# seanrjohnson/protein_gibbs_sampler

Measured on AMD Instinct MI355X. Metric: sampled positions/sec (whole node), ESM-1b L=256 B=256 Gibbs, higher is better.
Workload: dtype bf16; 1 GPU; ESM_sampler ESM-1b (33 layers, d=1280) Gibbs: 256 chains in total, 256 per GPU x L=256 (T=258), P=25 positions per chain per iteration, mask=True top_k=0 temperature=1.0 burnin=inf; bf16 MFMA operands, fp32 accumulate + fp32 residual stream; synthetic weights N(0,0.025), embeddings N(0,0.3), LayerNorm jitter 0.1 (logit std ~10); global_batch=256, seq_len=256, parallelism=chains sharded 1-way (contiguous blocks), 1 RCCL all-gather at the end, n_layers=33

## Files before the change

protein_gibbs_sampler_amd/csrc/attention.hip:

```cpp
#include <stdlib.h>

#include "attn_frag.h"

PG_OPS_BEGIN


#ifdef PG_ATT_PROF
__device__ unsigned long long* pg_att_prof;
#define PG_T(slot, i)                                                                                              \
  do {                                                                                                             \
    if ((slot) < 8 && (threadIdx.x & 63) == 0)                                                                     \
      pg_att_prof[(((size_t)blockIdx.x * 4 + (threadIdx.x >> 6)) * 8 + (slot)) * 8 + (i)] = __builtin_readcyclecounter(); \
  } while (0)
#else
#define PG_T(slot, i)
#endif

constexpr int attention_occupancy(int maxkb, int hd) { return hd == 64 ? (maxkb <= 18 ? 2 : 1) : 2; }
constexpr int attention_resident32(int kb) { return kb <= 20 ? 4 : (kb <= 26 ? 3 : 2); }
template <int MAXKB, bool PADMASK, bool BIASKV = false, bool SPLIT = false, int HD = 64>
__global__ __launch_bounds__(256, attention_occupancy(MAXKB, HD)) void attention_kernel(const bf16_t* __restrict__ qkv, bf16_t* __restrict__ ctx, int T,
                                                       int H, int ld_qkv_, int ld_ctx_, int k_off, int v_off,
                                                       SeqLayout sl, const int32_t* __restrict__ key_tok, int pad_idx,
                                                       const bf16_t* __restrict__ bias_kv, int split_from = 0, int split = 1) {
  constexpr int ROW = HD * 2, NKK = HD / 32, NDB = HD / 16;
  __shared__ __attribute__((aligned(16))) char smem[2 * MAXKB * 16 * ROW + (PADMASK ? MAXKB * 16 : 0)];
  char* Ks = smem;
  char* Vs = smem + MAXKB * 16 * ROW;
  char* padf = smem + 2 * MAXKB * 16 * ROW;

  const int tid = threadIdx.x, lane = tid & 63, wave = tid >> 6;
  PG_T(7, 0);
  int pair = blockIdx.x, qb_first = wave, qb_step = 4;
  if (SPLIT && (int)blockIdx.x >= split_from) {
    const int u = blockIdx.x - split_from;
    pair = split_from + u / split;
    qb_first = u % split + split * wave;
    qb_step = 4 * split;
  }
  const int seq = pair / H, h = pair % H;
  const size_t row0 = (size_t)(seq / sl.inner_count) * sl.outer_rows + (size_t)(seq % sl.inner_count) * sl.inner_rows;
  const size_t ld_qkv = (size_t)ld_qkv_ * sl.row_step, ld_ctx = (size_t)ld_ctx_ * sl.row_step;
  const bf16_t* base = qkv + row0 * ld_qkv_ + h * HD;
  const int Tk = T + (BIASKV ? 1 : 0);
  constexpr int nkc = MAXKB / 2;

  stage_kv<MAXKB * 16, 256, BIASKV, HD>(Ks, Vs, tid, base, ld_qkv, k_off, v_off, 0, T, bias_kv + h * HD, bias_kv + (H + h) * HD);
  if (PADMASK) {
    for (int key = tid; key < MAXKB * 16; key += 256)
      padf[key] = (key < T && key_tok[row0 + (size_t)key * sl.row_step] == pad_idx) ? 1 : 0;
  }
  PG_T(7, 1);
  __syncthreads();
  PG_T(7, 2);

  const int fr = lane & 15, fq = lane >> 4;
  const int nqb = (T + 15) >> 4;
  bf16x8 qf[NKK], qn[NKK];
  auto load_q = [&](int qb, bf16x8 (&dst)[NKK]) {
    int qrow = qb * 16 + fr;
    if (qrow >= T) qrow = T - 1;
#pragma unroll
    for (int kk = 0; kk < NKK; ++kk) dst[kk] = *(const bf16x8*)(base + (size_t)qrow * ld_qkv + kk * 32 + fq * 8);
  };
  if (qb_first < nqb) load_q(qb_first, qf);
  for (int qb = qb_first; qb < nqb; qb += qb_step) {
    if (qb + qb_step < nqb) load_q(qb + qb_step, qn);
    PG_T(qb >> 2, 0);

    f32x4 st[MAXKB];
    {
      constexpr int CH = (MAXKB % 6 == 0) ? 6 : (MAXKB % 4 == 0 ? 4 : 2);
      bf16x8 kbuf[2][CH][NKK];
      auto load_chunk = [&](int ch, bf16x8 (&dst)[CH][NKK]) {
#pragma unroll
        for (int u = 0; u < CH; ++u) {
#if defined(PG_ATT_PROF) && PG_ATT_ABL == 1
          const int krow = (ch * CH + (u > 0 ? 0 : u)) * 16 + fr;
          if (u > 0) { for (int kk = 0; kk < NKK; ++kk) dst[u][kk] = dst[0][kk]; continue; }
#else
          const int krow = (ch * CH + u) * 16 + fr;
#endif
#pragma unroll
          for (int kk = 0; kk < NKK; ++kk) dst[u][kk] = k_frag<HD>(Ks, krow, kk, fq);
        }
      };
// ... 42 lines not shown
#pragma unroll
        for (int db = 0; db < NDB; ++db) {
#if defined(PG_ATT_PROF) && PG_ATT_ABL == 2
          if (db > 0) { dst[db] = dst[0]; continue; }
#endif
#pragma unroll
          for (int hh = 0; hh < 2; ++hh) dst[db].h[hh] = vt_half<HD>(Vs, (2 * c + hh) * 16, db, fr, fq);
        }
      };
      load_v(0, vbuf[0]);
      if (nkc > 1) load_v(1, vbuf[1]);
#pragma unroll
      for (int c = 0; c < nkc; ++c) {
        if (c + 2 < nkc) load_v(c + 2, vbuf[(c + 2) % 3]);
        const bf16x8 pf = p_frag(st[2 * c], st[2 * c + 1]);
        __builtin_amdgcn_sched_barrier(0);
#pragma unroll
        for (int db = 0; db < NDB; ++db) o[db] = mfma_op16(vbuf[c % 3][db].v, pf, o[db]);
        __builtin_amdgcn_sched_barrier(0);
      }
    }
    PG_T(qb >> 2, 3);
    const int q = qb * 16 + fr;
    if (q < T) store_ctx(o, inv, ctx + row0 * ld_ctx_ + (size_t)q * ld_ctx + h * HD + fq * 4);
    qf[0] = qn[0];
    if constexpr (NKK == 2) qf[1] = qn[1];
    PG_T(qb >> 2, 4);
  }
  PG_T(7, 3);
}

template <int MAXKB, int OCC, bool PADMASK, bool BIASKV, int HD = 64>
__global__ __launch_bounds__(256, OCC) void attention_long_kernel(const bf16_t* __restrict__ qkv, bf16_t* __restrict__ ctx, int T,
                                                               int H, int ld_qkv_, int ld_ctx_, int k_off, int v_off,
                                                               SeqLayout sl, int n_qchunk, const int32_t* __restrict__ key_tok_,
                                                               int pad_idx, const bf16_t* __restrict__ bias_kv_) {
  const int32_t* __restrict__ key_tok = PADMASK ? key_tok_ : nullptr;
  const bf16_t* __restrict__ bias_kv = BIASKV ? bias_kv_ : nullptr;
  constexpr int tpad = MAXKB * 16, nkc = MAXKB / 2;
  constexpr int ROW = HD * 2, NKK = HD / 32, NDB = HD / 16;
  __shared__ __attribute__((aligned(16))) char smem[2 * tpad * ROW + (PADMASK ? tpad : 0)];
  char* Ks = smem;
  char* Vs = smem + tpad * ROW;
  char* padf = smem + 2 * tpad * ROW;
  const int tid = threadIdx.x, lane = tid & 63, wave = tid >> 6;
  const int qc = blockIdx.x % n_qchunk, sh = blockIdx.x / n_qchunk;
  const int seq = sh / H, h = sh % H;
// ... 111 lines not shown
  dim3 grid((unsigned)(n_seq * H)), block(256);
  static const int fine_ladder = env_int("PGIBBS_ATTN_LADDER", 1);
  const int kb = attention_rung(T + (bias_kv ? 1 : 0), fine_ladder && !bias_kv);
  static const int split_on = env_int("PGIBBS_ATTN_SPLIT", 1);
  int split_from = 0, split = 1;
  if (split_on && !key_tok && !bias_kv && sl.row_step == 1 && T >= 64 && kb) {
    const long pairs = n_seq * H, slots = (long)device_cu_count() * (head_dim == 64 ? (kb <= 20 ? 2 : 1) : attention_resident32(kb));
    const long rem = pairs % slots;
    const int nqb = (T + 15) / 16;
    int sp = rem ? (int)(slots / rem) : 1;
    if (sp > 4) sp = 4;
    if (sp > nqb / 4) sp = nqb / 4;
    if (sp >= 2) {
      split = sp;
      split_from = (int)(pairs - rem);
      grid = dim3((unsigned)(split_from + rem * sp));
    }
  }
  switch (kb) {
#define PG_RUNG(KB)                                                                                                          \
  case KB:                                                                                                                   \
    if (head_dim == 64)                                                                                                      \
      launch_rung<KB, 64>(key_tok, bias_kv, split > 1, grid, s, qkv, ctx, T, H, ld_qkv, ld_ctx, k_off, v_off, sl, key_tok,   \
                          pad_idx, bias_kv, split_from, split);                                                              \
    else                                                                                                                     \
      launch_rung<KB, 32>(key_tok, false, split > 1, grid, s, qkv, ctx, T, H, ld_qkv, ld_ctx, k_off, v_off, sl, key_tok,     \
                          pad_idx, bias_kv, split_from, split);                                                              \
    break;
    PG_RUNG(2) PG_RUNG(4) PG_RUNG(6) PG_RUNG(8) PG_RUNG(10) PG_RUNG(12) PG_RUNG(14) PG_RUNG(16) PG_RUNG(18) PG_RUNG(20)
    PG_RUNG(22) PG_RUNG(24) PG_RUNG(26) PG_RUNG(28) PG_RUNG(30) PG_RUNG(32) PG_RUNG(34) PG_RUNG(36)
#undef PG_RUNG
    default: {
      const int n_qchunk = (T + 63) / 64;
      if (n_seq * H * n_qchunk > 0x7fffffff) return fail(1, "attention: too many sequences");
      const dim3 g((unsigned)(n_seq * H * n_qchunk));
#define PG_ATT_LONG(P, B) hipLaunchKernelGGL((attention_long_kernel<18, 2, P, B>), g, block, 0, s, qkv, ctx, T, H, ld_qkv, ld_ctx, k_off, v_off, sl, n_qchunk, key_tok, pad_idx, bias_kv)
#define PG_ATT_LONG32(P) hipLaunchKernelGGL((attention_long_kernel<18, 2, P, false, 32>), g, block, 0, s, qkv, ctx, T, H, ld_qkv, ld_ctx, k_off, v_off, sl, n_qchunk, key_tok, pad_idx, bias_kv)
      if (head_dim == 32) {
        if (key_tok) PG_ATT_LONG32(true);
        else PG_ATT_LONG32(false);
      } else if (key_tok && bias_kv) PG_ATT_LONG(true, true);
      else if (key_tok) PG_ATT_LONG(true, false);
      else if (bias_kv) PG_ATT_LONG(false, true);
      else PG_ATT_LONG(false, false);
#undef PG_ATT_LONG32
#undef PG_ATT_LONG
    }
  }
  PG_HIP(hipGetLastError());
  return 0;
}

PG_OPS_END
```

protein_gibbs_sampler_amd/csrc/engine.h:

```cpp
#pragma once
#include <map>
#include <string>
#include <vector>

#include "kernels.h"

namespace pg {

#define OPS(fn, ...) (precision == PG_PREC_F16 ? opf16::fn(__VA_ARGS__) : opbf16::fn(__VA_ARGS__))

struct DevBuf {
  void* p = nullptr;
  size_t bytes = 0;
  int ensure(size_t need, hipStream_t s);
  void release();
  template <typename T> T* as() const { return (T*)p; }
};

struct Prof {
  struct Rec { int cls; hipEvent_t a, b; std::string kernels; };
  bool on = false;
  std::vector<Rec> recs;
  std::vector<hipEvent_t> pool;
  size_t used = 0;
// ... 24 lines not shown
struct MsaLayer {
  LnW ln_row, ln_col;
  DenseW row_qkv, row_out, col_qkv, col_out;
  FfnW ffn;
  DenseW col_qkv_hm;
};

struct Engine {
  pg_model_config cfg;
  int device = 0;
  int precision = 0;
  hipStream_t own_stream = nullptr, stream = nullptr;
  std::vector<void*> owned;

  float *embed = nullptr, *pos = nullptr, *msa_pos = nullptr, *embed_out = nullptr;
  float embed_scale() const { return cfg.arch == PG_ARCH_ESM1 ? sqrtf((float)cfg.d_model) : 1.0f; }
  LnW ln_before, ln_after, head_ln;
  DenseW head_dense;
  float* head_bias = nullptr;
  std::vector<EsmLayer> esm_layers;
  std::vector<MsaLayer> msa_layers;

  DevBuf x, h, qkv, ctx, ffn, sel_h, sel_g, logits, d_tokens, d_idx, d_samp_tok, d_samp_logits, d_rowmap, scratch;
  DevBuf x_sel, ctx_sel, h_sel, ffn_sel;
  int resid_gemm_ln(const bf16_t* a, const DenseW& W, float* x, int M_rows, int64_t M_real, int lda, const LnW& ln, bf16_t* h,
                    float* ws = nullptr, size_t ws_bytes = 0, int prof_class = PC_GEMM, int colmajor_R = 0, int colmajor_C = 0);
  DevBuf tmp_idx, tmp_out;
  DevBuf splitk;
  bool esm_pad_in_batch = false;
  float* splitk_ws(int rows, int n, int K, int64_t batch_rows);
  int64_t job_items = 0;
  int64_t order_items = 0;
  int64_t job_batch(int64_t B) const { return order_items > 0 ? order_items : (job_items > B ? job_items : B); }
  int64_t batch_rows_for(int64_t B, int64_t rows_per_item) const { return job_batch(B) * rows_per_item; }
  int64_t batch_rows = 0;
  int sel_gemm_rows(int64_t n_sel, int64_t Np) const;
  DevBuf d_iter;
  PgChainLayerW* chain_layers = nullptr;
  DevBuf chain_sync, chain_part;
  unsigned* chain_err = nullptr;
  int chain_check();
  bool chain_disabled = false, chain_retry = false;
  struct ChainCall {
    int32_t* d_tok; int B, T; const int32_t* d_idx; int n_iters, P; pg_sample_params sp; float* lg; int32_t* st; size_t snap_off;
  };
  std::vector<ChainCall> chain_log;
  bool chain_replay_ok = false;
// ... 10 lines not shown
  int64_t stat_graph_captures = 0, stat_graph_replays = 0;
  DevBuf ffn_f32, scores;
  bool strict() const { return precision == PG_PREC_FP32; }
  bool esm1() const { return cfg.arch == PG_ARCH_ESM1; }
  bool esm2() const { return cfg.arch == PG_ARCH_ESM2; }
  bool esm_family() const { return cfg.arch == PG_ARCH_ESM1B || cfg.arch == PG_ARCH_ESM1 || cfg.arch == PG_ARCH_ESM2; }
  int head_dim = 64;
  float* rope_tab = nullptr;
  int rope_rows = 0;
  int rope(void* qkv_rows, int64_t M, int T);
  int dense3(const bf16_t* x3, const DenseW& W, float* out, int Mp, bool accumulate);
  int dense3_gelu(const bf16_t* x3, const DenseW& W, int Mp, const DenseW* next = nullptr);
  bool dense3_wants_dup(const DenseW& W, int Mp, bool gelu = false) const;
  Prof prof;

  ~Engine();
  int init(const pg_model_config* c, const pg_tensor* tensors, int n_tensors, int device_ordinal, int precision);

  int size_activations(int64_t Mp);
  int ffn_block(const DenseW& out, const FfnW& F, const LnW* next_ln, int Mi, int64_t M);
  int ffn_strict(const FfnW& F, int Mi, int64_t M);
  bool prune_last(int64_t n_draws, int64_t token_rows) const;
  int pruned_tail(const DenseW& out, const FfnW& F, const int32_t* sel_idx, const int32_t* sel_row_map, int P, int width, int64_t n_sel,
                  const int32_t* d_iter, int Ni, bool ln_in_gemm);
  int esm_trunk(const int32_t* d_tok, int B, int T, const int32_t* sel_idx, int P, int64_t n_sel, const int32_t* d_iter);
  int head(const int32_t* d_idx, const int32_t* d_row_map, int P, int width, int64_t n_sel, float* d_logits,
           const float* x_src = nullptr);
  int trunk(const int32_t* d_tok, int B, int R, int C, const int32_t* sel_idx = nullptr, const int32_t* sel_row_map = nullptr, int P = 0,
            int64_t n_sel = 0, const int32_t* d_iter = nullptr);
  int masked_logits(int32_t* d_tok, int B, int R, int C, const int32_t* idx, const int32_t* mask_map, const int32_t* sel_map,
                    int64_t n_rows, int P, bool mask, int mask_idx, float* lg, const int32_t* dit = nullptr);
  int esm_gibbs_device(int32_t* d_tok, int B, int T, const int32_t* d_idx, int n_iters, int P, const pg_sample_params* sp,
                       float* d_samp_logits, int32_t* d_samp_tok);
  int msa_trunk(const int32_t* d_tok, int B, int R, int C, const int32_t* sel_idx, const int32_t* sel_row_map, int P, int64_t n_sel);
  int msa_gibbs_device(int32_t* d_tok, int B, int R, int C, const int32_t* d_idx, int n_iters, int P,
                       const pg_sample_params* sp, float* d_samp_logits, int32_t* d_samp_tok);
  int msa_single_device(int32_t* d_tok, int B, int R, int C, int mask_row, int target_row, const int32_t* d_step_idx,
                        const int32_t* step_sample_flag_host, int n_steps, int P_max, const pg_sample_params* sp,
                        float* d_samp_logits, int32_t* d_samp_tok);

  template <typename F> int timed(int cls, F&& f);
};

std::vector<float> rope_table(int rows, int hd = 64);

struct TensorMap {
  std::map<std::string, const pg_tensor*> m;
// ... 9 lines not shown
```

protein_gibbs_sampler_amd/csrc/engine.hip:

```cpp
#include "engine.h"

#include <math.h>
#include <stdlib.h>
#include <string.h>

#include "gemm_epilogue.h"

namespace pg {

static thread_local std::string g_last_error;
void set_error(const std::string& msg) { g_last_error = msg; }
int fail(int code, const std::string& msg) {
  g_last_error = msg;
  return code;
}
const char* last_error_cstr() { return g_last_error.c_str(); }

static thread_local std::string g_noted;
void note_kernel(const char* label, long tiles, int splits) {
  if (g_noted.size() > 512) return;
  if (!g_noted.empty()) g_noted += " + ";
  g_noted += label;
  if (tiles >= 0) g_noted += " " + std::to_string(tiles) + "t";
  if (splits > 1) g_noted += " x" + std::to_string(splits) + "k";
// ... 50 lines not shown
  int rc = f();
  PG_HIP(hipEventRecord(b, stream));
  prof.recs.push_back({cls, a, b, noted_kernels()});
  return rc;
}

const float* TensorMap::get(const std::string& name, int64_t numel, std::string& err) const {
  auto it = m.find(name);
  if (it == m.end()) {
    err = "missing tensor '" + name + "'";
    return nullptr;
  }
  if (it->second->numel != numel) {
    err = "tensor '" + name + "' has " + std::to_string(it->second->numel) + " elements, expected " + std::to_string(numel);
    return nullptr;
  }
  return it->second->data;
}

Engine::~Engine() {
  if (device >= 0) (void)hipSetDevice(device);
  for (void* p : owned) (void)hipFree(p);
  DevBuf* bufs[] = {&x, &h, &qkv, &ctx, &ffn, &sel_h, &sel_g, &logits, &d_tokens, &d_idx, &d_samp_tok, &d_samp_logits,
                    &d_rowmap, &scratch, &d_iter, &tmp_idx, &tmp_out, &x_sel, &ctx_sel, &h_sel, &ffn_sel, &ffn_f32, &scores, &splitk,
                    &chain_sync, &chain_part, &chain_snap};
  for (DevBuf* b : bufs) b->release();
  if (chain_err) (void)hipHostFree(chain_err);
  if (range_err) (void)hipHostFree(range_err);
  prof.destroy();
  if (graph_exec) (void)hipGraphExecDestroy(graph_exec);
  if (own_stream) (void)hipStreamDestroy(own_stream);
}

namespace {
struct Uploader {
  Engine* e;
  const TensorMap* tm;
  const int precision;
  std::string err;

  float* f32(const std::string& name, int64_t numel) {
    const float* src = tm->get(name, numel, err);
    if (!src) return nullptr;
    void* d = nullptr;
    if (hipMalloc(&d, (size_t)numel * 4) != hipSuccess) { err = "hipMalloc failed for " + name; return nullptr; }
    e->owned.push_back(d);
    if (hipMemcpy(d, src, (size_t)numel * 4, hipMemcpyHostToDevice) != hipSuccess) { err = "H2D failed for " + name; return nullptr; }
// ... 319 lines not shown
  int rc;
  if ((rc = timed(PC_LN, [&] { return OPS(launch_layernorm_bf16, stream, X, F.ln.g, F.ln.b, H3, M, cfg.d_model, cfg.layer_norm_eps, true, 0, 0, dense3_wants_dup(F.fc1, Mi, true)); }))) return rc;
  if ((rc = dense3_gelu(H3, F.fc1, Mi, &F.fc2))) return rc;
  return dense3(ffn.as<bf16_t>(), F.fc2, X, Mi, true);
}

int Engine::ffn_block(const DenseW& out, const FfnW& F, const LnW* next_ln, int Mi, int64_t M) {
  const int d = cfg.d_model, f = cfg.d_ffn;
  float* X = x.as<float>();
  bf16_t* Hh = h.as<bf16_t>();
  bf16_t* FFN = ffn.as<bf16_t>();
  int rc;
  if ((rc = resid_gemm_ln(ctx.as<bf16_t>(), out, X, Mi, M, d, F.ln, Hh, nullptr, 0, PC_GEMM_OUT))) return rc;
  if ((rc = timed(PC_GEMM_FC1, [&] { return OPS(launch_gemm_bf16, stream, Hh, F.fc1.w, F.fc1.b, FFN, Mi, f, d, d, d, f, EPI_BF16_GELU, nullptr, 0, (int)M); }))) return rc;
  if (next_ln) return resid_gemm_ln(FFN, F.fc2, X, Mi, M, f, *next_ln, Hh, splitk_ws(Mi, d, f, batch_rows), splitk.bytes, PC_GEMM_FC2);
  return timed(PC_GEMM_FC2, [&] { return OPS(launch_gemm_bf16, stream, FFN, F.fc2.w, F.fc2.b, X, Mi, d, f, f, f, d, EPI_F32_RESID, splitk_ws(Mi, d, f, batch_rows), splitk.bytes, (int)M); });
}

bool Engine::prune_last(int64_t n_draws, int64_t token_rows) const {
  static const int prune = env_int("PGIBBS_PRUNE_LAST", 1);
  return prune && !strict() && n_draws > 0 && 2 * n_draws < token_rows;
}

int Engine::pruned_tail(const DenseW& out, const FfnW& F, const int32_t* sel_idx, const int32_t* sel_row_map, int P, int width,
                        int64_t n_sel, const int32_t* d_iter_, int Ni, bool ln_in_gemm) {
  const int d = cfg.d_model, f = cfg.d_ffn;
  const float eps = cfg.layer_norm_eps;
  const int64_t Np = round_up64(n_sel, kRowPad);
  int rc;
  if ((rc = x_sel.ensure((size_t)Np * d * 4, stream)) || (rc = ctx_sel.ensure((size_t)Np * d * 2, stream)) ||
      (rc = h_sel.ensure((size_t)Np * d * 2, stream)) || (rc = ffn_sel.ensure((size_t)Np * f * 2, stream))) return rc;
  float* XS = x_sel.as<float>();
  bf16_t* FS = ffn_sel.as<bf16_t>();
  rc = timed(PC_HEAD, [&] {
    int r2 = launch_gather_rows(stream, x.as<float>(), XS, sel_idx, sel_row_map, P, width, n_sel, d * 4, d_iter_);
    if (r2) return r2;
    return launch_gather_rows(stream, ctx.as<bf16_t>(), ctx_sel.as<bf16_t>(), sel_idx, sel_row_map, P, width, n_sel, d * 2, d_iter_);
  });
  if (rc) return rc;
  if ((rc = timed(PC_GEMM, [&] { return OPS(launch_gemm_bf16, stream, ctx_sel.as<bf16_t>(), out.w, out.b, XS, Ni, d, d, d, d, d, EPI_F32_RESID); }))) return rc;
  if (ln_in_gemm && gemm_ln_skinny_ok(Ni, f, d)) {
    if ((rc = timed(PC_GEMM, [&] { return OPS(launch_gemm_ln_skinny, stream, XS, d, F.ln.g, F.ln.b, eps, F.fc1.w, F.fc1.b, FS, Ni, f, d, d, f, EPI_BF16_GELU); }))) return rc;
  } else {
    if ((rc = timed(PC_LN, [&] { return OPS(launch_layernorm_bf16, stream, XS, F.ln.g, F.ln.b, h_sel.as<bf16_t>(), n_sel, d, eps); }))) return rc;
    if ((rc = timed(PC_GEMM, [&] { return OPS(launch_gemm_bf16, stream, h_sel.as<bf16_t>(), F.fc1.w, F.fc1.b, FS, Ni, f, d, d, d, f, EPI_BF16_GELU); }))) return rc;
  }
  return timed(PC_GEMM, [&] { return OPS(launch_gemm_bf16, stream, FS, F.fc2.w, F.fc2.b, XS, Ni, d, f, f, f, d, EPI_F32_RESID, splitk_ws(Ni, d, f, batch_rows), splitk.bytes); });
}

int Engine::trunk(const int32_t* d_tok, int B, int R, int C, const int32_t* sel_idx, const int32_t* sel_row_map, int P, int64_t n_sel,
                  const int32_t* d_iter_) {
  return cfg.arch == PG_ARCH_MSA1B ? msa_trunk(d_tok, B, R, C, sel_idx, sel_row_map, P, n_sel) : esm_trunk(d_tok, B, C, sel_idx, P, n_sel, d_iter_);
}

int Engine::esm_trunk(const int32_t* d_tok, int B, int T, const int32_t* sel_idx, int P, int64_t n_sel, const int32_t* d_iter_) {
  const int d = cfg.d_model, f = cfg.d_ffn;
  const int64_t M = (int64_t)B * T;
  const int64_t Mp = round_up64(M, kRowPad);
  int rc;
// ... 38 lines not shown
  bool attn_done = false;
  if (ln_in_gemm && chain_layers && !chain_disabled && !esm_pad_in_batch && T <= 32 && M <= Mi && OPS(chain_trunk_ok, Mi, d, f, cfg.n_heads)) {
    if ((rc = chain_sync.ensure(OPS(chain_trunk_sync_bytes), stream)) || (rc = chain_part.ensure(OPS(chain_trunk_part_bytes, Mi, d), stream))) return rc;
    PgChainTrunkArgs ca;
    ca.layers = chain_layers; ca.n_layers = cfg.n_layers; ca.partial_last = sel_idx ? 1 : 0; ca.B = B; ca.T = T;
    ca.x = X; ca.qkv = QKV; ca.ctx = CTX; ca.ffn = FFN; ca.part = chain_part.as<float>(); ca.sync = chain_sync.as<unsigned>();
    ca.err = chain_err; ca.eps = eps;
    rc = timed(PC_GEMM, [&] { return OPS(launch_chain_trunk, stream, ca, Mi, d); });
    if (rc == kChainTrunkUnfit) {
      chain_disabled = true;
    } else if (rc) {
      return rc;
    } else {
      static const int fault_at = env_int("PGIBBS_CHAIN_TRUNK_FAULT", 0);
      static int launches = 0;
      if (fault_at > 0 && ++launches == fault_at) *chain_err = 1;
      if (!sel_idx) return PG_OK;
      l_first = cfg.n_layers - 1;
      attn_done = true;
    }
  }
  for (int l = l_first; l < cfg.n_layers; ++l) {
    const EsmLayer& L = esm_layers[l];
    if (attn_done) {
    } else if (ln_in_gemm) {
      if ((rc = timed(PC_GEMM, [&] { return OPS(launch_gemm_ln_skinny, stream, X, d, L.ln1.g, L.ln1.b, eps, L.qkv.w, L.qkv.b, QKV, Mi, 3 * d, d, d, 3 * d, EPI_BF16); }))) return rc;
    } else {
      if ((rc = timed(PC_GEMM_QKV, [&] { return OPS(launch_gemm_bf16, stream, Hh, L.qkv.w, L.qkv.b, QKV, Mi, 3 * d, d, d, d, 3 * d, EPI_BF16); }))) return rc;
    }
    if (!attn_done && (rc = rope(QKV, M, T))) return rc;
    if (!attn_done)
      if ((rc = timed(PC_ATTN, [&] { return OPS(launch_attention_bf16, stream, QKV, CTX, B, T, cfg.n_heads, 3 * d, d, d, 2 * d, esm_pad_in_batch ? d_tok : nullptr, cfg.pad_idx, L.bias_kv16, head_dim); }))) return rc;
    const bool last = l == cfg.n_layers - 1;
    if (sel_idx && last) return pruned_tail(L.out, L.ffn, sel_idx, nullptr, P, T, n_sel, d_iter_, sel_gemm_rows(n_sel, round_up64(n_sel, kRowPad)), ln_in_gemm);
    if (!ln_in_gemm) {
      if ((rc = ffn_block(L.out, L.ffn, last ? nullptr : &esm_layers[l + 1].ln1, Mi, M))) return rc;
      continue;
    }
    const FfnW& F = L.ffn;
    if ((rc = timed(PC_GEMM, [&] { return OPS(launch_gemm_bf16, stream, CTX, L.out.w, L.out.b, X, Mi, d, d, d, d, d, EPI_F32_RESID); }))) return rc;
    if ((rc = timed(PC_GEMM, [&] { return OPS(launch_gemm_ln_skinny, stream, X, d, F.ln.g, F.ln.b, eps, F.fc1.w, F.fc1.b, FFN, Mi, f, d, d, f, EPI_BF16_GELU); }))) return rc;
    if ((rc = timed(PC_GEMM, [&] { return OPS(launch_gemm_bf16, stream, FFN, F.fc2.w, F.fc2.b, X, Mi, d, f, f, f, d, EPI_F32_RESID, splitk_ws(Mi, d, f, batch_rows), splitk.bytes, (int)M); }))) return rc;
  }
  return PG_OK;
}

// ... 310 lines not shown
```

protein_gibbs_sampler_amd/csrc/kernels_ops.inc:

```
int launch_gemm_bf16(hipStream_t s, const bf16_t* X, const bf16_t* W, const float* bias, void* out, int M, int N, int K,
                     int ldx, int ldw, int ldo, int epi, float* ws = nullptr, size_t ws_bytes = 0, int m_live = 0);
int gemm_splitk_splits(int K);
size_t gemm_splitk_ws_bytes(int M, int N, int K);
int launch_gemm_bf16_variant(hipStream_t s, const bf16_t* X, const bf16_t* W, const float* bias, void* out, int M, int N,
                             int K, int ldx, int ldw, int ldo, int epi, int variant, float* ws = nullptr, size_t ws_bytes = 0,
                             int m_live = 0);

bool gemm_ln_skinny_ok(int M, int N, int K);
int launch_gemm_ln_skinny(hipStream_t s, const float* X, int ldx, const float* gamma, const float* beta, float eps, const bf16_t* W,
                          const float* bias, void* out, int M, int N, int K, int ldw, int ldo, int epi);
bool chain_trunk_ok(int M, int d_model, int d_ffn, int n_heads);
size_t chain_trunk_sync_bytes();
size_t chain_trunk_part_bytes(int M, int d_model);
int launch_chain_trunk(hipStream_t s, const PgChainTrunkArgs& a, int M, int d_model);
int launch_gemm_big(hipStream_t s, const bf16_t* X, const bf16_t* W, const float* bias, void* out, int M, int N, int K, int ldx,
                    int ldw, int ldo, int epi, int m_live = 0);
bool gemm_ladder_has(int epi, int h);
int launch_gemm_ladder(hipStream_t s, const bf16_t* X, const bf16_t* W, const float* bias, void* out, int m_live, int m_rows, int h,
                       int N, int K, int ldx, int ldw, int ldo, int epi);
bool gemm_rowln_ok(int m_rows, int N, int K);
int launch_gemm_rowln(hipStream_t s, const bf16_t* A, const bf16_t* W, const float* bias, float* x, const float* gamma,
                      const float* beta, bf16_t* h, int m_live, int m_rows, int K, int lda, int ldw, float eps, int colmajor_R = 0,
                      int colmajor_C = 0, int abl = 0);
void gemm_plan_text(int M, int N, int K, int epi, int variant, bool have_ws, int m_live, int n_cu, std::string* text);
void gemm_big_geometry(int M, int N, int K, int* m_main_panels, int* tail_rows);
int launch_gemm_w16(hipStream_t s, const bf16_t* X, const bf16_t* W, const float* bias, void* out, int M, int N, int K, int ldx,
                    int ldw, int ldo, int epi, int abl = 0, int tail_rows = 0);
int launch_gemm_split3(hipStream_t s, const bf16_t* X3, const bf16_t* W3, const float* bias, void* out, int M, int N, int K, int ldo,
                       int epi);
bool gemm_split3_fused(int M, int N, int K, int epi);
int launch_gemm_split3_w16(hipStream_t s, const bf16_t* X3, const bf16_t* W3, const float* bias, void* out, int M, int N, int K,
                           int ldo, int epi);

int launch_attention_bf16(hipStream_t s, const bf16_t* qkv, bf16_t* ctx, int B, int T, int H, int ld_qkv, int ld_ctx,
                          int k_off, int v_off, const int32_t* key_tok = nullptr, int pad_idx = -1, const bf16_t* bias_kv = nullptr,
                          int head_dim = 64);
int launch_attention_seq_bf16(hipStream_t s, const bf16_t* qkv, bf16_t* ctx, int64_t n_seq, int T, int H, int ld_qkv,
                              int ld_ctx, int k_off, int v_off, SeqLayout sl, const int32_t* key_tok = nullptr,
                              int pad_idx = -1, const bf16_t* bias_kv = nullptr, int head_dim = 64);
size_t msa_row_split_scratch_bytes(int B, int R, int C, int H, int order_bh);
int launch_msa_row_attention_bf16(hipStream_t s, const bf16_t* qkv, bf16_t* ctx, int B, int R, int C, int H, int ld_qkv,
                                  int ld_ctx, int k_off, int v_off, float scale, float* partial = nullptr,
                                  size_t partial_bytes = 0, int order_bh = 0);

int launch_embed_ln(hipStream_t s, const int32_t* tokens, const float* embed, const float* pos, const float* msa_pos,
                    const float* gamma, const float* beta, float* x, int64_t n_tok, int T, int d, int pad_idx,
                    int mask_idx, int token_dropout, int rows_per_msa, float eps,
                    const float* gamma2 = nullptr, const float* beta2 = nullptr, bf16_t* h2 = nullptr,
                    float embed_scale = 1.0f);
int launch_rope(hipStream_t s, void* qkv, bool f32, const float* table, int table_rows, int64_t M, int T, int H, int ld,
                int head_dim = 64);
int launch_layernorm_bf16(hipStream_t s, const float* x, const float* gamma, const float* beta, bf16_t* h, int64_t M,
                          int d, float eps, bool split3 = false,
                          int colmajor_R = 0, int colmajor_C = 0,
                          bool split3_dup = true);
bool colattn_ok(int R, int d_model, int n_heads);
int launch_gemm_colattn(hipStream_t s, const bf16_t* X, const bf16_t* W, const float* bias, bf16_t* ctx, int B, int R, int C, int H,
                        int d, int ld_ctx);
int launch_headmajor_qkv(hipStream_t s, const bf16_t* w, const float* b, bf16_t* w2, float* b2, int H, int K);
int launch_layernorm_f32(hipStream_t s, const float* x, const float* gamma, const float* beta, float* y, int64_t M, int d,
                         float eps);
int launch_gather_ln_bf16(hipStream_t s, const float* x, const int32_t* idx, const int32_t* row_map, int P, int width,
                          const float* gamma, const float* beta, bf16_t* h, int64_t n_sel, int d, float eps,
                          bool split3 = false);
int launch_split3_bf16(hipStream_t s, const float* src, bf16_t* dst, int64_t rows, int K, float scale, bool gelu, bool weight);
int launch_gelu_f32(hipStream_t s, float* p, int64_t n);
int launch_attention_f32(hipStream_t s, const float* qkv, bf16_t* ctx, int split_d, int64_t n_seq, int T, int H,
                         int ld_qkv, int ld_ctx, int k_off, int v_off, SeqLayout sl, const int32_t* key_tok = nullptr,
                         int pad_idx = -1, const float* bias_kv = nullptr,
                         int head_dim = 64);
static inline int msa_row_scores_ld(int C) { return (C + 3) & ~3; }
int launch_msa_row_attention_f32(hipStream_t s, const float* qkv, float* scores, bf16_t* ctx, int split_d, int B, int R,
                                 int C, int H, int ld_qkv, int ld_ctx, int k_off, int v_off, float scale,
                                 const int32_t* tok = nullptr, int pad_idx = -1);
// ... 9 lines not shown
```

protein_gibbs_sampler_amd/csrc/rope.hip:

```cpp
#include "kernels.h"

PG_OPS_BEGIN

constexpr int kRopePass16 = 4, kRopePass16Wide = 5;
constexpr int kRopePass32 = 8, kRopePass32Wide = 10;
constexpr int kRopeHeads = 32, kRopeHeadsWide = 40;
constexpr int kRopePass16Hd32 = 2, kRopePass32Hd32 = 4;

__device__ __forceinline__ void rope_pair(float& lo, float& hi, float c, float s) {
  const float a = lo, b = hi;
  lo = __fsub_rn(__fmul_rn(a, c), __fmul_rn(b, s));
  hi = __fadd_rn(__fmul_rn(b, c), __fmul_rn(a, s));
}

__device__ __forceinline__ void rope_word16(uint32_t& wl, uint32_t& wh, float c0, float s0, float c1, float s1) {
  float l0 = op16_to_f32((bf16_t)(wl & 0xffff)), l1 = op16_to_f32((bf16_t)(wl >> 16));
  float h0 = op16_to_f32((bf16_t)(wh & 0xffff)), h1 = op16_to_f32((bf16_t)(wh >> 16));
  rope_pair(l0, h0, c0, s0);
  rope_pair(l1, h1, c1, s1);
  wl = pack_op2(l0, l1);
  wh = pack_op2(h0, h1);
}

template <int NP, int HD = 64>
__global__ __launch_bounds__(256) void rope16_kernel(bf16_t* __restrict__ qkv, const float* __restrict__ tab, int M, int T, int H,
                                                    int ld) {
  constexpr int LPH = HD / 16;
  const int lane = threadIdx.x & 63;
  const int stride = (int)gridDim.x * 4;
  const int slots = 2 * LPH * H;
  const int c = lane & (LPH - 1);
  for (int row = (int)blockIdx.x * 4 + (int)(threadIdx.x >> 6); row < M; row += stride) {
    const float4* tr = (const float4*)(tab + (size_t)(row % T) * HD);
    uint4* base = (uint4*)(qkv + (size_t)row * ld);
    uint4 lo[NP], hi[NP];
#pragma unroll
    for (int i = 0; i < NP; ++i) {
      const int s = lane + 64 * i;
      if (s < slots) {
        const uint4* p = base + (s / LPH) * (2 * LPH) + c;
        lo[i] = p[0];
        hi[i] = p[LPH];
      }
    }
    const float4 ca = tr[2 * c], cb = tr[2 * c + 1], sa = tr[HD / 8 + 2 * c], sb = tr[HD / 8 + 2 * c + 1];
#pragma unroll
    for (int i = 0; i < NP; ++i) {
      const int s = lane + 64 * i;
      if (s < slots) {
        rope_word16(lo[i].x, hi[i].x, ca.x, sa.x, ca.y, sa.y);
        rope_word16(lo[i].y, hi[i].y, ca.z, sa.z, ca.w, sa.w);
        rope_word16(lo[i].z, hi[i].z, cb.x, sb.x, cb.y, sb.y);
        rope_word16(lo[i].w, hi[i].w, cb.z, sb.z, cb.w, sb.w);
        uint4* p = base + (s / LPH) * (2 * LPH) + c;
        p[0] = lo[i];
        p[LPH] = hi[i];
      }
// ... 61 lines not shown
  if (head_dim == 64 && (H < 1 || H > kRopeHeadsWide)) return fail(1, "rope: 1..40 heads of 64 (d_model <= 2560)");
  if (head_dim == 32 && (H < 1 || H > kRopeHeads)) return fail(1, "rope: 1..32 heads of 32 (d_model <= 1024)");
  if (T < 1 || T > table_rows) return fail(1, "rope: sequence longer than the cos / sin table");
  if (ld < 3 * H * head_dim || ld % (f32 ? 4 : 8)) return fail(1, "rope: rows must hold [q | k | v] and keep 16-byte alignment");
  if (M == 0) return 0;
  if (M > 0x7fffffff - 4 * 8 * 1024) return fail(1, "rope: too many rows");
  if (head_dim == 32) {
    static const int occ16h = rope_occupancy(rope16_kernel<kRopePass16Hd32, 32>);
    static const int occ32h = rope_occupancy(rope32_kernel<kRopePass32Hd32, 32>);
    return f32 ? rope_launch(rope32_kernel<kRopePass32Hd32, 32>, occ32h, s, (float*)qkv, table, M, T, H, ld)
               : rope_launch(rope16_kernel<kRopePass16Hd32, 32>, occ16h, s, (bf16_t*)qkv, table, M, T, H, ld);
  }
  static const int occ16 = rope_occupancy(rope16_kernel<kRopePass16>);
  static const int occ32 = rope_occupancy(rope32_kernel<kRopePass32>);
  static const int occ16w = rope_occupancy(rope16_kernel<kRopePass16Wide>);
  static const int occ32w = rope_occupancy(rope32_kernel<kRopePass32Wide>);
  const bool wide = H > kRopeHeads;
  if (f32) return wide ? rope_launch(rope32_kernel<kRopePass32Wide>, occ32w, s, (float*)qkv, table, M, T, H, ld)
                       : rope_launch(rope32_kernel<kRopePass32>, occ32, s, (float*)qkv, table, M, T, H, ld);
  return wide ? rope_launch(rope16_kernel<kRopePass16Wide>, occ16w, s, (bf16_t*)qkv, table, M, T, H, ld)
              : rope_launch(rope16_kernel<kRopePass16>, occ16, s, (bf16_t*)qkv, table, M, T, H, ld);
}

PG_OPS_END
```

Before: 71570 sampled positions/s.

## Prune last-layer queries to sampled positions in QKV and attention

In the final layer, only the sampled positions' outputs are needed. The last layer now computes K/V for all rows but Q only for the gathered selected rows. Attention then runs over just those P queries per sequence through a new listed-queries attention kernel variant. ctx_sel is written directly, so the later gather is skipped. This removes roughly a third of the last layer's QKV GEMM work and most of its attention, at the cost of an extra gather, a small GEMM and added code paths.

Result: no change. 71860 sampled positions/s, median of 6 (+0.4%).

```diff
diff --git a/protein_gibbs_sampler_amd/csrc/attention.hip b/protein_gibbs_sampler_amd/csrc/attention.hip
--- a/protein_gibbs_sampler_amd/csrc/attention.hip
+++ b/protein_gibbs_sampler_amd/csrc/attention.hip
@@ -18,11 +18,13 @@
 
 constexpr int attention_occupancy(int maxkb, int hd) { return hd == 64 ? (maxkb <= 18 ? 2 : 1) : 2; }
 constexpr int attention_resident32(int kb) { return kb <= 20 ? 4 : (kb <= 26 ? 3 : 2); }
-template <int MAXKB, bool PADMASK, bool BIASKV = false, bool SPLIT = false, int HD = 64>
+template <int MAXKB, bool PADMASK, bool BIASKV = false, bool SPLIT = false, int HD = 64, bool SEL = false>
 __global__ __launch_bounds__(256, attention_occupancy(MAXKB, HD)) void attention_kernel(const bf16_t* __restrict__ qkv, bf16_t* __restrict__ ctx, int T,
                                                        int H, int ld_qkv_, int ld_ctx_, int k_off, int v_off,
                                                        SeqLayout sl, const int32_t* __restrict__ key_tok, int pad_idx,
-                                                       const bf16_t* __restrict__ bias_kv, int split_from = 0, int split = 1) {
+                                                       const bf16_t* __restrict__ bias_kv, int split_from = 0, int split = 1,
+                                                       const bf16_t* __restrict__ q_sel = nullptr, int P = 0) {
+  static_assert(!SEL || (!PADMASK && !SPLIT), "the listed-queries form: no <pad> mask (the Gibbs path), whole pairs");
   constexpr int ROW = HD * 2, NKK = HD / 32, NDB = HD / 16;
   __shared__ __attribute__((aligned(16))) char smem[2 * MAXKB * 16 * ROW + (PADMASK ? MAXKB * 16 : 0)];
   char* Ks = smem;
@@ -55,13 +57,16 @@
   PG_T(7, 2);
 
   const int fr = lane & 15, fq = lane >> 4;
-  const int nqb = (T + 15) >> 4;
+  const int nq = SEL ? P : T;
+  const int nqb = (nq + 15) >> 4;
+  const bf16_t* qbase = SEL ? q_sel + (size_t)seq * P * ld_ctx_ + h * HD : base;
+  const size_t ld_q = SEL ? (size_t)ld_ctx_ : ld_qkv;
   bf16x8 qf[NKK], qn[NKK];
   auto load_q = [&](int qb, bf16x8 (&dst)[NKK]) {
     int qrow = qb * 16 + fr;
-    if (qrow >= T) qrow = T - 1;
-#pragma unroll
-    for (int kk = 0; kk < NKK; ++kk) dst[kk] = *(const bf16x8*)(base + (size_t)qrow * ld_qkv + kk * 32 + fq * 8);
+    if (qrow >= nq) qrow = nq - 1;
+#pragma unroll
+    for (int kk = 0; kk < NKK; ++kk) dst[kk] = *(const bf16x8*)(qbase + (size_t)qrow * ld_q + kk * 32 + fq * 8);
   };
   if (qb_first < nqb) load_q(qb_first, qf);
   for (int qb = qb_first; qb < nqb; qb += qb_step) {
@@ -150,7 +155,11 @@
     }
     PG_T(qb >> 2, 3);
     const int q = qb * 16 + fr;
-    if (q < T) store_ctx(o, inv, ctx + row0 * ld_ctx_ + (size_t)q * ld_ctx + h * HD + fq * 4);
+    if (SEL) {
+      if (q < P) store_ctx(o, inv, ctx + ((size_t)seq * P + q) * ld_ctx_ + h * HD + fq * 4);
+    } else if (q < T) {
+      store_ctx(o, inv, ctx + row0 * ld_ctx_ + (size_t)q * ld_ctx + h * HD + fq * 4);
+    }
     qf[0] = qn[0];
     if constexpr (NKK == 2) qf[1] = qn[1];
     PG_T(qb >> 2, 4);
@@ -308,10 +317,10 @@
   case KB:                                                                                                                   \
     if (head_dim == 64)                                                                                                      \
       launch_rung<KB, 64>(key_tok, bias_kv, split > 1, grid, s, qkv, ctx, T, H, ld_qkv, ld_ctx, k_off, v_off, sl, key_tok,   \
-                          pad_idx, bias_kv, split_from, split);                                                              \
+                          pad_idx, bias_kv, split_from, split, (const bf16_t*)nullptr, 0);                                   \
     else                                                                                                                     \
       launch_rung<KB, 32>(key_tok, false, split > 1, grid, s, qkv, ctx, T, H, ld_qkv, ld_ctx, k_off, v_off, sl, key_tok,     \
-                          pad_idx, bias_kv, split_from, split);                                                              \
+                          pad_idx, bias_kv, split_from, split, (const bf16_t*)nullptr, 0);                                   \
     break;
     PG_RUNG(2) PG_RUNG(4) PG_RUNG(6) PG_RUNG(8) PG_RUNG(10) PG_RUNG(12) PG_RUNG(14) PG_RUNG(16) PG_RUNG(18) PG_RUNG(20)
     PG_RUNG(22) PG_RUNG(24) PG_RUNG(26) PG_RUNG(28) PG_RUNG(30) PG_RUNG(32) PG_RUNG(34) PG_RUNG(36)
@@ -337,4 +346,47 @@
   return 0;
 }
 
+bool attention_sel_ok(int T, bool bias_kv, int head_dim) {
+  static const int fine_ladder = env_int("PGIBBS_ATTN_LADDER", 1);
+  if (head_dim != 64 && (head_dim != 32 || bias_kv)) return false;
+  return T > 0 && attention_rung(T + (bias_kv ? 1 : 0), fine_ladder && !bias_kv) != 0;
+}
+
+template <int KB, int HD, class... Args>
+static void launch_rung_sel(bool bias, dim3 grid, hipStream_t s, Args... args) {
+  auto go = [&](auto* kernel) { hipLaunchKernelGGL(kernel, grid, dim3(256), 0, s, args...); };
+  if constexpr (coarse_rung(KB) && HD == 64) {
+    if (bias) return go(attention_kernel<KB, false, true, false, HD, true>);
+  }
+  go(attention_kernel<KB, false, false, false, HD, true>);
+}
+
+int launch_attention_sel_bf16(hipStream_t s, const bf16_t* q_sel, const bf16_t* qkv, bf16_t* ctx_sel, int B, int T, int H, int P,
+                              int ld_qkv, int ld_sel, int k_off, int v_off, const bf16_t* bias_kv, int head_dim) {
+  if (!attention_sel_ok(T, bias_kv != nullptr, head_dim)) return fail(1, "attention (listed queries): no whole-sequence kernel for this shape");
+  if (B == 0 || P == 0) return 0;
+  if (P < 0 || (int64_t)B * H > 0x7fffffff) return fail(1, "attention (listed queries): bad sizes");
+  static const int fine_ladder = env_int("PGIBBS_ATTN_LADDER", 1);
+  const int kb = attention_rung(T + (bias_kv ? 1 : 0), fine_ladder && !bias_kv);
+  const dim3 grid((unsigned)((int64_t)B * H));
+  const SeqLayout sl = {1, T, 0, 1};
+  switch (kb) {
+#define PG_RUNG(KB)                                                                                                          \
+  case KB:                                                                                                                   \
+    if (head_dim == 64)                                                                                                      \
+      launch_rung_sel<KB, 64>(bias_kv, grid, s, qkv, ctx_sel, T, H, ld_qkv, ld_sel, k_off, v_off, sl, (const int32_t*)nullptr, \
+                              -1, bias_kv, 0, 1, q_sel, P);                                                                  \
+    else                                                                                                                     \
+      launch_rung_sel<KB, 32>(false, grid, s, qkv, ctx_sel, T, H, ld_qkv, ld_sel, k_off, v_off, sl, (const int32_t*)nullptr, \
+                              -1, bias_kv, 0, 1, q_sel, P);                                                                  \
+    break;
+    PG_RUNG(2) PG_RUNG(4) PG_RUNG(6) PG_RUNG(8) PG_RUNG(10) PG_RUNG(12) PG_RUNG(14) PG_RUNG(16) PG_RUNG(18) PG_RUNG(20)
+    PG_RUNG(22) PG_RUNG(24) PG_RUNG(26) PG_RUNG(28) PG_RUNG(30) PG_RUNG(32) PG_RUNG(34) PG_RUNG(36)
+#undef PG_RUNG
+    default: return fail(1, "attention (listed queries): no rung");
+  }
+  PG_HIP(hipGetLastError());
+  return 0;
+}
+
 PG_OPS_END
diff --git a/protein_gibbs_sampler_amd/csrc/engine.h b/protein_gibbs_sampler_amd/csrc/engine.h
--- a/protein_gibbs_sampler_amd/csrc/engine.h
+++ b/protein_gibbs_sampler_amd/csrc/engine.h
@@ -70,7 +70,7 @@
   std::vector<MsaLayer> msa_layers;
 
   DevBuf x, h, qkv, ctx, ffn, sel_h, sel_g, logits, d_tokens, d_idx, d_samp_tok, d_samp_logits, d_rowmap, scratch;
-  DevBuf x_sel, ctx_sel, h_sel, ffn_sel;
+  DevBuf x_sel, ctx_sel, h_sel, ffn_sel, q_sel;
   int resid_gemm_ln(const bf16_t* a, const DenseW& W, float* x, int M_rows, int64_t M_real, int lda, const LnW& ln, bf16_t* h,
                     float* ws = nullptr, size_t ws_bytes = 0, int prof_class = PC_GEMM, int colmajor_R = 0, int colmajor_C = 0);
   DevBuf tmp_idx, tmp_out;
@@ -127,7 +127,9 @@
   int ffn_strict(const FfnW& F, int Mi, int64_t M);
   bool prune_last(int64_t n_draws, int64_t token_rows) const;
   int pruned_tail(const DenseW& out, const FfnW& F, const int32_t* sel_idx, const int32_t* sel_row_map, int P, int width, int64_t n_sel,
-                  const int32_t* d_iter, int Ni, bool ln_in_gemm);
+                  const int32_t* d_iter, int Ni, bool ln_in_gemm, bool have_ctx_sel = false);
+  bool prune_last_q(int B, int T, int P, int64_t n_sel, int Mi, bool bias_kv) const;
+  int pruned_qkv_attn(const EsmLayer& L, const int32_t* sel_idx, int B, int T, int P, int64_t n_sel, const int32_t* d_iter, int Mi);
   int esm_trunk(const int32_t* d_tok, int B, int T, const int32_t* sel_idx, int P, int64_t n_sel, const int32_t* d_iter);
   int head(const int32_t* d_idx, const int32_t* d_row_map, int P, int width, int64_t n_sel, float* d_logits,
            const float* x_src = nullptr);
diff --git a/protein_gibbs_sampler_amd/csrc/engine.hip b/protein_gibbs_sampler_amd/csrc/engine.hip
--- a/protein_gibbs_sampler_amd/csrc/engine.hip
+++ b/protein_gibbs_sampler_amd/csrc/engine.hip
@@ -96,7 +96,7 @@
   if (device >= 0) (void)hipSetDevice(device);
   for (void* p : owned) (void)hipFree(p);
   DevBuf* bufs[] = {&x, &h, &qkv, &ctx, &ffn, &sel_h, &sel_g, &logits, &d_tokens, &d_idx, &d_samp_tok, &d_samp_logits,
-                    &d_rowmap, &scratch, &d_iter, &tmp_idx, &tmp_out, &x_sel, &ctx_sel, &h_sel, &ffn_sel, &ffn_f32, &scores, &splitk,
+                    &d_rowmap, &scratch, &d_iter, &tmp_idx, &tmp_out, &x_sel, &ctx_sel, &h_sel, &ffn_sel, &q_sel, &ffn_f32, &scores, &splitk,
                     &chain_sync, &chain_part, &chain_snap};
   for (DevBuf* b : bufs) b->release();
   if (chain_err) (void)hipHostFree(chain_err);
@@ -462,8 +462,38 @@
   return prune && !strict() && n_draws > 0 && 2 * n_draws < token_rows;
 }
 
+bool Engine::prune_last_q(int B, int T, int P, int64_t n_sel, int Mi, bool bias_kv) const {
+  static const int on = env_int("PGIBBS_PRUNE_LAST_Q", 1);
+  return on && !strict() && !esm_pad_in_batch && P > 0 && n_sel == (int64_t)B * P && Mi > 48 && OPS(attention_sel_ok, T, bias_kv, head_dim);
+}
+
+int Engine::pruned_qkv_attn(const EsmLayer& L, const int32_t* sel_idx, int B, int T, int P, int64_t n_sel, const int32_t* d_iter_, int Mi) {
+  const int d = cfg.d_model, H = cfg.n_heads;
+  const int64_t Np = round_up64(n_sel, kRowPad);
+  int rc;
+  if ((rc = h_sel.ensure((size_t)Np * d * 2, stream)) || (rc = q_sel.ensure((size_t)Np * d * 2, stream)) ||
+      (rc = ctx_sel.ensure((size_t)Np * d * 2, stream))) return rc;
+  bf16_t* Hh = h.as<bf16_t>();
+  bf16_t* QKV = qkv.as<bf16_t>();
+  bf16_t* HS = h_sel.as<bf16_t>();
+  bf16_t* QS = q_sel.as<bf16_t>();
+  const int Nq = n_sel > 256 ? (int)Np : round_up((int)n_sel, 64);
+  if ((rc = timed(PC_GEMM_QKV, [&] { return OPS(launch_gemm_bf16, stream, Hh, L.qkv.w + (size_t)d * d, L.qkv.b + d, QKV + d, Mi, 2 * d, d, d, d, 3 * d, EPI_BF16); }))) return rc;
+  if ((rc = timed(PC_HEAD, [&] { return launch_gather_rows(stream, Hh, HS, sel_idx, nullptr, P, T, n_sel, d * 2, d_iter_); }))) return rc;
+  if ((rc = timed(PC_GEMM_QKV, [&] { return OPS(launch_gemm_bf16, stream, HS, L.qkv.w, L.qkv.b, QS, Nq, d, d, d, d, d, EPI_BF16); }))) return rc;
+  if (esm2()) {
+    rc = timed(PC_ROPE, [&] {
+      int r2 = OPS(launch_rope_rows, stream, QKV + d, rope_tab, rope_rows, (int64_t)B * T, T, H, 3 * d, nullptr, nullptr, head_dim);
+      if (r2) return r2;
+      return OPS(launch_rope_rows, stream, QS, rope_tab, rope_rows, n_sel, T, H, d, sel_idx, d_iter_, head_dim);
+    });
+    if (rc) return rc;
+  }
+  return timed(PC_ATTN, [&] { return OPS(launch_attention_sel_bf16, stream, QS, QKV, ctx_sel.as<bf16_t>(), B, T, H, P, 3 * d, d, d, 2 * d, L.bias_kv16, head_dim); });
+}
+
 int Engine::pruned_tail(const DenseW& out, const FfnW& F, const int32_t* sel_idx, const int32_t* sel_row_map, int P, int width,
-                        int64_t n_sel, const int32_t* d_iter_, int Ni, bool ln_in_gemm) {
+                        int64_t n_sel, const int32_t* d_iter_, int Ni, bool ln_in_gemm, bool have_ctx_sel) {
   const int d = cfg.d_model, f = cfg.d_ffn;
   const float eps = cfg.layer_norm_eps;
   const int64_t Np = round_up64(n_sel, kRowPad);
@@ -474,7 +504,7 @@
   bf16_t* FS = ffn_sel.as<bf16_t>();
   rc = timed(PC_HEAD, [&] {
     int r2 = launch_gather_rows(stream, x.as<float>(), XS, sel_idx, sel_row_map, P, width, n_sel, d * 4, d_iter_);
-    if (r2) return r2;
+    if (r2 || have_ctx_sel) return r2;
     return launch_gather_rows(stream, ctx.as<bf16_t>(), ctx_sel.as<bf16_t>(), sel_idx, sel_row_map, P, width, n_sel, d * 2, d_iter_);
   });
   if (rc) return rc;
@@ -559,6 +589,10 @@
   }
   for (int l = l_first; l < cfg.n_layers; ++l) {
     const EsmLayer& L = esm_layers[l];
+    if (sel_idx && l == cfg.n_layers - 1 && !attn_done && !ln_in_gemm && prune_last_q(B, T, P, n_sel, Mi, L.bias_kv16 != nullptr)) {
+      if ((rc = pruned_qkv_attn(L, sel_idx, B, T, P, n_sel, d_iter_, Mi))) return rc;
+      return pruned_tail(L.out, L.ffn, sel_idx, nullptr, P, T, n_sel, d_iter_, sel_gemm_rows(n_sel, round_up64(n_sel, kRowPad)), ln_in_gemm, true);
+    }
     if (attn_done) {
     } else if (ln_in_gemm) {
       if ((rc = timed(PC_GEMM, [&] { return OPS(launch_gemm_ln_skinny, stream, X, d, L.ln1.g, L.ln1.b, eps, L.qkv.w, L.qkv.b, QKV, Mi, 3 * d, d, d, 3 * d, EPI_BF16); }))) return rc;
diff --git a/protein_gibbs_sampler_amd/csrc/kernels_ops.inc b/protein_gibbs_sampler_amd/csrc/kernels_ops.inc
--- a/protein_gibbs_sampler_amd/csrc/kernels_ops.inc
+++ b/protein_gibbs_sampler_amd/csrc/kernels_ops.inc
@@ -38,6 +38,9 @@
 int launch_attention_seq_bf16(hipStream_t s, const bf16_t* qkv, bf16_t* ctx, int64_t n_seq, int T, int H, int ld_qkv,
                               int ld_ctx, int k_off, int v_off, SeqLayout sl, const int32_t* key_tok = nullptr,
                               int pad_idx = -1, const bf16_t* bias_kv = nullptr, int head_dim = 64);
+bool attention_sel_ok(int T, bool bias_kv, int head_dim);
+int launch_attention_sel_bf16(hipStream_t s, const bf16_t* q_sel, const bf16_t* qkv, bf16_t* ctx_sel, int B, int T, int H, int P,
+                              int ld_qkv, int ld_sel, int k_off, int v_off, const bf16_t* bias_kv = nullptr, int head_dim = 64);
 size_t msa_row_split_scratch_bytes(int B, int R, int C, int H, int order_bh);
 int launch_msa_row_attention_bf16(hipStream_t s, const bf16_t* qkv, bf16_t* ctx, int B, int R, int C, int H, int ld_qkv,
                                   int ld_ctx, int k_off, int v_off, float scale, float* partial = nullptr,
@@ -50,6 +53,8 @@
                     float embed_scale = 1.0f);
 int launch_rope(hipStream_t s, void* qkv, bool f32, const float* table, int table_rows, int64_t M, int T, int H, int ld,
                 int head_dim = 64);
+int launch_rope_rows(hipStream_t s, bf16_t* buf, const float* table, int table_rows, int64_t M, int T, int heads, int ld,
+                     const int32_t* pos_idx = nullptr, const int32_t* d_iter = nullptr, int head_dim = 64);
 int launch_layernorm_bf16(hipStream_t s, const float* x, const float* gamma, const float* beta, bf16_t* h, int64_t M,
                           int d, float eps, bool split3 = false,
                           int colmajor_R = 0, int colmajor_C = 0,
diff --git a/protein_gibbs_sampler_amd/csrc/rope.hip b/protein_gibbs_sampler_amd/csrc/rope.hip
--- a/protein_gibbs_sampler_amd/csrc/rope.hip
+++ b/protein_gibbs_sampler_amd/csrc/rope.hip
@@ -33,6 +33,52 @@
   for (int row = (int)blockIdx.x * 4 + (int)(threadIdx.x >> 6); row < M; row += stride) {
     const float4* tr = (const float4*)(tab + (size_t)(row % T) * HD);
     uint4* base = (uint4*)(qkv + (size_t)row * ld);
+    uint4 lo[NP], hi[NP];
+#pragma unroll
+    for (int i = 0; i < NP; ++i) {
+      const int s = lane + 64 * i;
+      if (s < slots) {
+        const uint4* p = base + (s / LPH) * (2 * LPH) + c;
+        lo[i] = p[0];
+        hi[i] = p[LPH];
+      }
+    }
+    const float4 ca = tr[2 * c], cb = tr[2 * c + 1], sa = tr[HD / 8 + 2 * c], sb = tr[HD / 8 + 2 * c + 1];
+#pragma unroll
+    for (int i = 0; i < NP; ++i) {
+      const int s = lane + 64 * i;
+      if (s < slots) {
+        rope_word16(lo[i].x, hi[i].x, ca.x, sa.x, ca.y, sa.y);
+        rope_word16(lo[i].y, hi[i].y, ca.z, sa.z, ca.w, sa.w);
+        rope_word16(lo[i].z, hi[i].z, cb.x, sb.x, cb.y, sb.y);
+        rope_word16(lo[i].w, hi[i].w, cb.z, sb.z, cb.w, sb.w);
+        uint4* p = base + (s / LPH) * (2 * LPH) + c;
+        p[0] = lo[i];
+        p[LPH] = hi[i];
+      }
+    }
+  }
+}
+
+template <int NP, int HD = 64>
+__global__ __launch_bounds__(256) void rope16_rows_kernel(bf16_t* __restrict__ buf, const float* __restrict__ tab, int M, int T, int heads,
+                                                         int ld, const int32_t* __restrict__ pos_idx,
+                                                         const int32_t* __restrict__ d_iter) {
+  constexpr int LPH = HD / 16;
+  const int lane = threadIdx.x & 63;
+  const int stride = (int)gridDim.x * 4;
+  const int slots = LPH * heads;
+  const int c = lane & (LPH - 1);
+  if (pos_idx && d_iter) pos_idx += (size_t)(*d_iter) * M;
+  for (int row = (int)blockIdx.x * 4 + (int)(threadIdx.x >> 6); row < M; row += stride) {
+    int pos = row % T;
+    if (pos_idx) {
+      pos = pos_idx[row];
+      pos = pos < 0 ? 0 : (pos & 0x3fffffff);
+      if (pos >= T) pos = 0;
+    }
+    const float4* tr = (const float4*)(tab + (size_t)pos * HD);
+    uint4* base = (uint4*)(buf + (size_t)row * ld);
     uint4 lo[NP], hi[NP];
 #pragma unroll
     for (int i = 0; i < NP; ++i) {
@@ -140,4 +186,22 @@
               : rope_launch(rope16_kernel<kRopePass16>, occ16, s, (bf16_t*)qkv, table, M, T, H, ld);
 }
 
+int launch_rope_rows(hipStream_t s, bf16_t* buf, const float* table, int table_rows, int64_t M, int T, int heads, int ld,
+                     const int32_t* pos_idx, const int32_t* d_iter, int head_dim) {
+  if (head_dim != 64 && head_dim != 32) return fail(1, "rope: head dimension " + std::to_string(head_dim) + ": the kernels are built for 64 and 32");
+  if (head_dim == 64 && (heads < 1 || heads > kRopeHeadsWide)) return fail(1, "rope: 1..40 heads of 64 (d_model <= 2560)");
+  if (head_dim == 32 && (heads < 1 || heads > kRopeHeads)) return fail(1, "rope: 1..32 heads of 32 (d_model <= 1024)");
+  if (T < 1 || T > table_rows) return fail(1, "rope: sequence longer than the cos / sin table");
+  if (ld < heads * head_dim || ld % 8) return fail(1, "rope: rows must hold the heads and keep 16-byte alignment");
+  if (M == 0) return 0;
+  if (M > 0x7fffffff - 4 * 8 * 1024) return fail(1, "rope: too many rows");
+  const int64_t need = (M + 3) / 4, resident = (int64_t)device_cu_count() * 4;
+  const dim3 grid((unsigned)(need < resident ? need : resident));
+  if (head_dim == 32) hipLaunchKernelGGL((rope16_rows_kernel<kRopePass16Hd32, 32>), grid, dim3(256), 0, s, buf, table, (int)M, T, heads, ld, pos_idx, d_iter);
+  else if (heads > kRopeHeads) hipLaunchKernelGGL((rope16_rows_kernel<kRopePass16Wide>), grid, dim3(256), 0, s, buf, table, (int)M, T, heads, ld, pos_idx, d_iter);
+  else hipLaunchKernelGGL((rope16_rows_kernel<kRopePass16>), grid, dim3(256), 0, s, buf, table, (int)M, T, heads, ld, pos_idx, d_iter);
+  PG_HIP(hipGetLastError());
+  return 0;
+}
+
 PG_OPS_END
```
